# TravisWheelerLab/BATH

Measured on NVIDIA B200. Metric: frameshift Forward GCUPS, higher is better.
Workload: dtype f32

## Files before the change

### bath_b200/csrc/bathgpu.cu

```cuda
#include <cuda_runtime.h>
#include <stdint.h>
#include <stdio.h>
#include <stdarg.h>
#include <string.h>
#include <stdlib.h>
#include <math.h>
#include <thread>
#include <vector>
#include <string>
#include <algorithm>
#include <mutex>
#include <memory>

#include "../../include/bathgpu.h"
#include "fs_parser.cuh"
#include "fs_parser_v3.cuh"
#include "fs_backward.cuh"
#include "fs_domain.cuh"
#include "orf_domain.cuh"
#include "orf_filters.cuh"
#include "orf_finder.cuh"
#include "bias_filter.cuh"
#include "microbench.cuh"
#include "launch.h"
// ... 56 lines not shown
struct FsProfileSet {
  int n = 0;
  std::vector<int> J, scan_steps, mw_scan_steps;
  std::vector<FsSetProfile> table;
  DevBuf arena, dtable, dwins, dwprof, dsc, dst, dcounter;
};

}

struct TargetSlot {
  DevBuf  dna_bytes, dna4, residues, cls;
  int64_t block_n = 0, nres = 0;
  bool    bytes_valid = false;
};
constexpr int kMaxSlots = 1 << 16;

struct bathgpu_ctx {
  int           device = 0;
  cudaDeviceProp prop{};
  cudaStream_t  stream = nullptr, copy_stream = nullptr, stream2 = nullptr;
  cudaStream_t  bulk_stream = nullptr;
  cudaEvent_t   chunk_ev[16] = {};
  cudaEvent_t   ev0 = nullptr, ev1 = nullptr;
  cudaEvent_t   sync_ev = nullptr;
  std::string   err;
  FsProfileImage fs3, fs5;
  FsProfileSet  set3, set5;
  std::vector<std::unique_ptr<TargetSlot>> slot;
  int           cur = 0;
  TargetSlot   &S() { return *slot[cur]; }
  TargetSlot   &slot_at(int i) { while ((int)slot.size() <= i) slot.emplace_back(new TargetSlot()); return *slot[i]; }
  DevBuf        wins, fwdsc, status, counter;
  int           nstaged = 0;
  DevBuf        scratch;
  DevBuf        fxmx, bxmx, lsf, lsb, xoff, dmocc, dbtot, detot, bcksc;
  int64_t       xrows = 0;
  bool          flt_loaded = false;
  bathgpu_filter_params flt{};
  int           flt_W = 0, flt_P = 0;
  DevBuf        f_rbv, f_rwv, f_twv, f_ddsum, f_nrb, orfs, fsc, fst, fwins, fnw;
  DevBuf        b_items, b_tables, b_out;
  DevBuf        o_tiles, o_cnt, o_base, o_blocks, o_first, o_tjb, o_null, o_meta, o_hits, o_counters;
  long long     o_nhits = 0, o_nres = 0;
  cudaEvent_t   o_ev[6] = {};
  float         o_ms[5] = {};
  long long     o_scored = 0, o_norf = 0;
  DevBuf        envs, dpp, doa, dfx, dppx, doax, dlsf, dfw, dbk, doasc, dnull2, dstat, dtoff, dtlen, dsteps, ddcell, dmxout;
  std::vector<long long> dom_xoff;
  std::vector<int>       dom_L;
  float         last_ms = 0.f;
  int           last_launches = 0;
};

static int fail(bathgpu_ctx *ctx, int code, const char *fmt, ...)
{
  char buf[512];
  va_list ap;
  va_start(ap, fmt);
  vsnprintf(buf, sizeof buf, fmt, ap);
  va_end(ap);
  if (ctx) ctx->err = buf;
  return code;
}

#define CUDA_TRY(ctx, call)                                                                      \
  do { cudaError_t e_ = (call);                                                                  \
// ... 766 lines not shown
  const long long p = (long long)blockIdx.x * blockDim.x + threadIdx.x;
  if (p >= n) return;
  const uint8_t comp[18] = { 3, 2, 1, 0, 4, 6, 5, 8, 7, 9, 10, 14, 13, 12, 11, 15, 16, 17 };
  const uint8_t c = src[n - p];
  dst[1 + p] = (c < 18) ? comp[c] : c;
  if (p == 0) { dst[0] = 255; dst[n + 1] = 255; }
}

extern "C" int bathgpu_revcomp_slot(bathgpu_ctx *ctx, int src, int dst)
{
  if (!ctx || src < 0 || src >= kMaxSlots || dst < 0 || dst >= kMaxSlots || src == dst) return fail(ctx, BATHGPU_EINVAL, "bad arguments to bathgpu_revcomp_slot");
  ctx->slot_at(std::max(src, dst));
  TargetSlot &A = *ctx->slot[src], &B = *ctx->slot[dst];
  if (A.block_n == 0) return fail(ctx, BATHGPU_EINVAL, "no block uploaded in slot %d", src);
  CUDA_TRY(ctx, enter(ctx));
  const long long n = A.block_n;
  const long long nwords = (n + 8 + 7) / 8 + 24;
  if (B.dna_bytes.reserve((size_t)n + 2) != BATHGPU_OK || B.dna4.reserve((size_t)nwords * 4) != BATHGPU_OK)
    return fail(ctx, BATHGPU_EMEM, "device allocation failed for a %lld-nt block", n);
  if (!A.bytes_valid) {
    unpack_dna4_kernel<<<(unsigned)(((n + 7) / 8 + 255) / 256), 256, 0, ctx->stream>>>(A.dna4.as<uint32_t>(), n, A.dna_bytes.as<uint8_t>());
    A.bytes_valid = true;
  }
  revcomp_kernel<<<(unsigned)((n + 255) / 256), 256, 0, ctx->stream>>>(A.dna_bytes.as<uint8_t>(), n, B.dna_bytes.as<uint8_t>());
  pack_dna4_kernel<<<(unsigned)((nwords + 255) / 256), 256, 0, ctx->stream>>>(B.dna_bytes.as<uint8_t>(), n, B.dna4.as<uint32_t>(), nwords);
  CUDA_TRY(ctx, cudaGetLastError());
  CUDA_TRY(ctx, wait_stream(ctx));
  B.block_n = n; B.nres = 0; B.bytes_valid = true;
  return BATHGPU_OK;
}


static cudaError_t dispatch_fwd(bool xmx, int J, const FsParserArgs &a, int sms, cudaStream_t s);

static int fs_fwd_block_impl(bathgpu_ctx *ctx, const uint8_t *dsq, const uint8_t *packed, int64_t n, const bathgpu_window *wins, int nwin,
                             const float xfE[2], float *fwdsc, int32_t *status)
{
  if (!ctx || (!dsq && !packed) || n < 1 || !wins || nwin < 1 || !xfE || !fwdsc || !status) return fail(ctx, BATHGPU_EINVAL, "bad arguments to bathgpu_fs_fwd_block");
  if (!ctx->fs3.loaded) return fail(ctx, BATHGPU_EINVAL, "3-codon profile not loaded");
  for (int w = 0; w < nwin; ++w)
    if (wins[w].L < 3 || wins[w].start < 1 || wins[w].start + wins[w].L - 1 > n)
      return fail(ctx, BATHGPU_EINVAL, "window %d (start %lld, L %d) is outside the block (n=%lld) or shorter than 3", w, (long long)wins[w].start, wins[w].L, (long long)n);
  CUDA_TRY(ctx, enter(ctx));
  if (!ctx->copy_stream) {
    CUDA_TRY(ctx, cudaStreamCreateWithFlags(&ctx->copy_stream, cudaStreamNonBlocking));
    CUDA_TRY(ctx, cudaStreamCreateWithFlags(&ctx->stream2, cudaStreamNonBlocking));
    for (auto &e : ctx->chunk_ev) CUDA_TRY(ctx, cudaEventCreateWithFlags(&e, cudaEventDisableTiming));
  }
  TargetSlot &S = ctx->S();
  const long long nwords = (n + 8 + 7) / 8 + 24;
  if (S.dna_bytes.reserve((size_t)n + 2) != BATHGPU_OK || S.dna4.reserve((size_t)nwords * 4) != BATHGPU_OK ||
      ctx->wins.reserve((size_t)nwin * sizeof(WindowDesc)) != BATHGPU_OK || ctx->fwdsc.reserve((size_t)nwin * 4) != BATHGPU_OK ||
      ctx->status.reserve((size_t)nwin * 4) != BATHGPU_OK || ctx->counter.reserve(64) != BATHGPU_OK)
    return fail(ctx, BATHGPU_EMEM, "device allocation failed");
  S.block_n = n; S.nres = 0; S.bytes_valid = (packed == nullptr);
  static_assert(sizeof(WindowDesc) == sizeof(bathgpu_window), "descriptor layouts must agree");
  bool in_order = true;
  for (int w = 1; w < nwin && in_order; ++w) in_order = wins[w - 1].start + wins[w - 1].L <= wins[w].start + wins[w].L;
  std::vector<int> order;
  std::vector<WindowDesc> sorted;
  std::vector<float> sc;
  std::vector<int> st;
  if (!in_order) {
    order.resize((size_t)nwin); sorted.resize((size_t)nwin); sc.resize((size_t)nwin); st.resize((size_t)nwin);
    for (int w = 0; w < nwin; ++w) order[w] = w;
    std::sort(order.begin(), order.end(), [&](int x, int y) { return wins[x].start + wins[x].L < wins[y].start + wins[y].L; });
// ... 3 lines not shown
  long long cuts[8]; int K = 0;
  {
    long long first = n / 85, p = 0;
    const int wave = ctx->prop.multiProcessorCount * 16;
    if (nwin > wave) first = std::min<long long>(std::max<long long>(first, hw[wave].start + hw[wave].L), std::max<long long>(first, n / 8));
    if (n < (4 << 20)) first = n;
    for (long long sz = std::max<long long>(first, 1 << 20); p < n && K < 7; sz *= 4) { p = std::min<long long>(n, (p + sz + 7) & ~7LL); cuts[K++] = p; }
    cuts[K - 1] = n;
  }
  cudaEvent_t *pack_ev = ctx->chunk_ev, *join_ev = ctx->chunk_ev + 8;
  for (int c = 0; c < K; ++c) {
    const long long p0 = c ? cuts[c - 1] : 0, p1 = cuts[c];
    if (packed) {
      CUDA_TRY(ctx, cudaMemcpyAsync(S.dna4.as<uint8_t>() + 4 + p0 / 2, packed + p0 / 2, (size_t)((p1 + 1) / 2 - p0 / 2), cudaMemcpyHostToDevice, ctx->copy_stream));
      {
        const long long b0 = (4 + p0 / 2) & ~127LL, b1 = 4 + (p1 + 1) / 2, lines = (b1 - b0 + 127) / 128;
        l2_prefetch_kernel<<<(unsigned)((lines + 255) / 256), 256, 0, ctx->copy_stream>>>(S.dna4.as<uint8_t>() + b0, b1 - b0);
      }
      if (p1 >= n) dna4_guards_kernel<<<1, 32, 0, ctx->copy_stream>>>(S.dna4.as<uint32_t>(), n);
      else if (c == 0) dna4_guards_kernel<<<1, 1, 0, ctx->copy_stream>>>(S.dna4.as<uint32_t>(), n);
    } else {
      CUDA_TRY(ctx, cudaMemcpyAsync(S.dna_bytes.as<uint8_t>() + 1 + p0, dsq + 1 + p0, (size_t)(p1 - p0), cudaMemcpyHostToDevice, ctx->copy_stream));
      const long long wlo = (c == 0) ? 0 : p0 / 8 + 1, whi = (p1 >= n) ? nwords : p1 / 8 + 1;
      if (whi > wlo)
        pack_dna4_range_kernel<<<(unsigned)((whi - wlo + 255) / 256), 256, 0, ctx->copy_stream>>>(S.dna_bytes.as<uint8_t>(), n, S.dna4.as<uint32_t>(), wlo, whi);
    }
    CUDA_TRY(ctx, cudaGetLastError());
    CUDA_TRY(ctx, cudaEventRecord(pack_ev[c], ctx->copy_stream));
  }
  CUDA_TRY(ctx, cudaMemcpyAsync(ctx->wins.p, hw, (size_t)nwin * sizeof(WindowDesc), cudaMemcpyHostToDevice, ctx->stream));
  CUDA_TRY(ctx, cudaMemsetAsync(ctx->counter.p, 0, 64, ctx->stream));
  CUDA_TRY(ctx, cudaEventRecord(ctx->ev0, ctx->stream));
  const FsProfileImage &im = ctx->fs3;
  int w0 = 0, launches = 0;
  for (int c = 0; c < K; ++c) {
    const long long ready_nt = (c == K - 1) ? n : 8 * (cuts[c] / 8);
    int w1 = w0;
    while (w1 < nwin && hw[w1].start + hw[w1].L - 1 <= ready_nt) ++w1;
    if (c == K - 1) w1 = nwin;
    if (w1 == w0) continue;
    cudaStream_t s = (launches & 1) ? ctx->stream2 : ctx->stream;
    if (launches == 1) CUDA_TRY(ctx, cudaStreamWaitEvent(ctx->stream2, ctx->ev0, 0));
    CUDA_TRY(ctx, cudaStreamWaitEvent(s, pack_ev[c], 0));
    FsParserArgs a{};
    a.emis = im.emis_fwd.as<float>(); a.cellc = im.cellc.as<float>(); a.dna4 = S.dna4.as<uint32_t>();
    a.wins = ctx->wins.as<WindowDesc>() + w0; a.nwin = w1 - w0; a.mpad = im.mpad; a.tEM = xfE[0]; a.tEL = xfE[1];
    a.fwdsc = ctx->fwdsc.as<float>() + w0; a.status = ctx->status.as<int>() + w0; a.xmx = nullptr; a.xoff = nullptr;
    a.counter = ctx->counter.as<int>() + launches; a.scan_steps = im.scan_steps; a.cellmw = im.cellmw.as<float>(); a.mw_scan_steps = im.mw_scan_steps;
    CUDA_TRY(ctx, dispatch_fwd(false, im.J, a, ctx->prop.multiProcessorCount, s));
    ++launches;
    w0 = w1;
  }
  if (launches > 1) {
    CUDA_TRY(ctx, cudaEventRecord(join_ev[0], ctx->stream2));
    CUDA_TRY(ctx, cudaStreamWaitEvent(ctx->stream, join_ev[0], 0));
  }
  CUDA_TRY(ctx, cudaEventRecord(ctx->ev1, ctx->stream));
  CUDA_TRY(ctx, cudaMemcpyAsync(in_order ? fwdsc : sc.data(), ctx->fwdsc.p, (size_t)nwin * 4, cudaMemcpyDeviceToHost, ctx->stream));
  CUDA_TRY(ctx, cudaMemcpyAsync(in_order ? status : st.data(), ctx->status.p, (size_t)nwin * 4, cudaMemcpyDeviceToHost, ctx->stream));
  CUDA_TRY(ctx, wait_stream(ctx));
  CUDA_TRY(ctx, cudaStreamSynchronize(ctx->copy_stream));
  if (!in_order) for (int w = 0; w < nwin; ++w) { fwdsc[order[w]] = sc[w]; status[order[w]] = st[w]; }
  CUDA_TRY(ctx, cudaEventElapsedTime(&ctx->last_ms, ctx->ev0, ctx->ev1));
  ctx->last_launches = launches;
  ctx->nstaged = 0;
  return BATHGPU_OK;
}

extern "C" int bathgpu_fs_fwd_block(bathgpu_ctx *ctx, const uint8_t *dsq, int64_t n, const bathgpu_window *wins, int nwin,
                                    const float xfE[2], float *fwdsc, int32_t *status)
{
  if (!dsq) return fail(ctx, BATHGPU_EINVAL, "bad arguments to bathgpu_fs_fwd_block");
  return fs_fwd_block_impl(ctx, dsq, nullptr, n, wins, nwin, xfE, fwdsc, status);
}

extern "C" int bathgpu_fs_fwd_block_packed4(bathgpu_ctx *ctx, const uint8_t *packed, int64_t n, const bathgpu_window *wins, int nwin,
                                            const float xfE[2], float *fwdsc, int32_t *status)
{
  if (!packed) return fail(ctx, BATHGPU_EINVAL, "bad arguments to bathgpu_fs_fwd_block_packed4");
  return fs_fwd_block_impl(ctx, nullptr, packed, n, wins, nwin, xfE, fwdsc, status);
}

static int fwd_version(int J)
{
  static const int forced = [] { const char *e = getenv("BATHGPU_FWD"); int x = e ? atoi(e) : 0; return (x == 3 || x == 4) ? x : 0; }();
  if (forced) return forced;
  return (J == 10) ? 4 : 3;
}

static cudaError_t dispatch_fwd(bool xmx, int J, const FsParserArgs &a, int sms, cudaStream_t s)
{
  cudaError_t e = cudaErrorInvalidValue;
  const int v = fwd_version(J);
#define X(S) if (launch_fs3_forward_##S(J, xmx, v, a, sms, s, &e)) return e;
  BATHGPU_FOR_EACH_SET(X)
#undef X
  return cudaErrorInvalidValue;
}

static int check_windows(bathgpu_ctx *ctx, const bathgpu_window *wins, int n)
{
  for (int w = 0; w < n; ++w) {
    if (wins[w].L < 3 || wins[w].start < 1 || wins[w].start + wins[w].L - 1 > ctx->S().block_n)
      return fail(ctx, BATHGPU_EINVAL, "window %d (start %lld, L %d) is outside the uploaded block (n=%lld) or shorter than 3",
                  w, (long long)wins[w].start, wins[w].L, (long long)ctx->S().block_n);
  }
  return BATHGPU_OK;
}

extern "C" int bathgpu_stage_windows(bathgpu_ctx *ctx, const bathgpu_window *wins, int n)
{
  if (!ctx || !wins || n < 1) return fail(ctx, BATHGPU_EINVAL, "bad arguments to bathgpu_stage_windows");
  if (ctx->S().block_n == 0)      return fail(ctx, BATHGPU_EINVAL, "no block uploaded");
  int st = check_windows(ctx, wins, n);
  if (st != BATHGPU_OK) return st;
  CUDA_TRY(ctx, enter(ctx));
  static_assert(sizeof(WindowDesc) == sizeof(bathgpu_window), "descriptor layouts must agree");
  if (ctx->wins.reserve((size_t)n * sizeof(WindowDesc)) != BATHGPU_OK || ctx->fwdsc.reserve((size_t)n * 4) != BATHGPU_OK ||
      ctx->status.reserve((size_t)n * 4) != BATHGPU_OK || ctx->counter.reserve(64) != BATHGPU_OK)
    return fail(ctx, BATHGPU_EMEM, "device allocation failed");
  CUDA_TRY(ctx, cudaMemcpyAsync(ctx->wins.p, wins, (size_t)n * sizeof(WindowDesc), cudaMemcpyHostToDevice, ctx->stream));
  CUDA_TRY(ctx, wait_stream(ctx));
  ctx->nstaged = n;
  return BATHGPU_OK;
}

extern "C" int bathgpu_fs_fwd_staged(bathgpu_ctx *ctx, const float xfE[2])
{
  if (!ctx || !xfE)          return fail(ctx, BATHGPU_EINVAL, "bad arguments to bathgpu_fs_fwd_staged");
  if (!ctx->fs3.loaded)      return fail(ctx, BATHGPU_EINVAL, "3-codon profile not loaded");
  if (ctx->nstaged < 1)      return fail(ctx, BATHGPU_EINVAL, "no windows staged");
  CUDA_TRY(ctx, enter(ctx));
  const FsProfileImage &im = ctx->fs3;
  FsParserArgs a{};
  a.emis = im.emis_fwd.as<float>(); a.cellc = im.cellc.as<float>(); a.dna4 = ctx->S().dna4.as<uint32_t>();
  a.wins = ctx->wins.as<WindowDesc>(); a.nwin = ctx->nstaged; a.mpad = im.mpad;
  a.tEM = xfE[0]; a.tEL = xfE[1];
  a.fwdsc = ctx->fwdsc.as<float>(); a.status = ctx->status.as<int>();
  a.xmx = nullptr; a.xoff = nullptr; a.counter = ctx->counter.as<int>(); a.scan_steps = im.scan_steps; a.cellmw = im.cellmw.as<float>(); a.mw_scan_steps = im.mw_scan_steps;

  CUDA_TRY(ctx, cudaMemsetAsync(ctx->counter.p, 0, 4, ctx->stream));
  CUDA_TRY(ctx, cudaEventRecord(ctx->ev0, ctx->stream));
  CUDA_TRY(ctx, dispatch_fwd(false, im.J, a, ctx->prop.multiProcessorCount, ctx->stream));
  CUDA_TRY(ctx, cudaEventRecord(ctx->ev1, ctx->stream));
  CUDA_TRY(ctx, wait_stream(ctx));
  CUDA_TRY(ctx, cudaEventElapsedTime(&ctx->last_ms, ctx->ev0, ctx->ev1));
  ctx->last_launches = 1;
  return BATHGPU_OK;
}

extern "C" int bathgpu_fetch_scores(bathgpu_ctx *ctx, float *fwdsc, int32_t *status, int n)
{
  if (!ctx || n < 1 || n > ctx->nstaged) return fail(ctx, BATHGPU_EINVAL, "bad arguments to bathgpu_fetch_scores");
  CUDA_TRY(ctx, enter(ctx));
  if (fwdsc)  CUDA_TRY(ctx, cudaMemcpyAsync(fwdsc,  ctx->fwdsc.p,  (size_t)n * 4, cudaMemcpyDeviceToHost, ctx->stream));
  if (status) CUDA_TRY(ctx, cudaMemcpyAsync(status, ctx->status.p, (size_t)n * 4, cudaMemcpyDeviceToHost, ctx->stream));
  CUDA_TRY(ctx, wait_stream(ctx));
  return BATHGPU_OK;
}

extern "C" int bathgpu_fs_fwd_windows(bathgpu_ctx *ctx, const bathgpu_window *wins, int n, const float xfE[2],
                                      float *fwdsc, int32_t *status)
{
  int st;
  if (!fwdsc || !status) return fail(ctx, BATHGPU_EINVAL, "bad arguments to bathgpu_fs_fwd_windows");
  if ((st = bathgpu_stage_windows(ctx, wins, n)) != BATHGPU_OK) return st;
  if ((st = bathgpu_fs_fwd_staged(ctx, xfE))     != BATHGPU_OK) return st;
  return bathgpu_fetch_scores(ctx, fwdsc, status, n);
}

static cudaError_t dispatch_bck(int J, const FsBackwardArgs &a, int sms, cudaStream_t s)
{
  cudaError_t e = cudaErrorInvalidValue;
#define X(S) if (launch_fs3_backward_##S(J, a, sms, s, &e)) return e;
  BATHGPU_FOR_EACH_SET(X)
#undef X
  return cudaErrorInvalidValue;
}

static int bck_decode_chunk(bathgpu_ctx *ctx, const bathgpu_window *wins, int n, const float xfE[2], const float xf5_loop[3],
                            const int64_t *out_offset, float *mocc, float *btot, float *etot,
                            float *fwdsc, float *bcksc, int32_t *status,
                            int64_t x_off0 = 0, float *fx_out = nullptr, float *bx_out = nullptr)
{
  const bool decode = (xf5_loop != nullptr);
  const FsProfileImage &im = ctx->fs3;
  std::vector<long long> xoff(n + 1, 0);
  for (int w = 0; w < n; ++w) xoff[w + 1] = xoff[w] + wins[w].L + 1;
  const size_t rows = (size_t)xoff[n];

  if (ctx->wins.reserve((size_t)n * sizeof(WindowDesc)) != BATHGPU_OK || ctx->fwdsc.reserve((size_t)n * 4) != BATHGPU_OK ||
      ctx->bcksc.reserve((size_t)n * 4) != BATHGPU_OK || ctx->status.reserve((size_t)n * 4) != BATHGPU_OK ||
      ctx->counter.reserve(64) != BATHGPU_OK || ctx->xoff.reserve((size_t)(n + 1) * 8) != BATHGPU_OK ||
      ctx->fxmx.reserve(rows * 24) != BATHGPU_OK || ctx->bxmx.reserve(rows * 24) != BATHGPU_OK ||
      ctx->lsf.reserve((rows + 2 * (size_t)n) * 4) != BATHGPU_OK || ctx->lsb.reserve((rows + 2 * (size_t)n) * 4) != BATHGPU_OK ||
      ctx->dmocc.reserve(rows * 4) != BATHGPU_OK || ctx->dbtot.reserve(rows * 4) != BATHGPU_OK || ctx->detot.reserve(rows * 4) != BATHGPU_OK)
    return fail(ctx, BATHGPU_EMEM, "device allocation failed for %d windows (%zu rows)", n, rows);
  CUDA_TRY(ctx, cudaMemcpyAsync(ctx->wins.p, wins, (size_t)n * sizeof(WindowDesc), cudaMemcpyHostToDevice, ctx->stream));
  CUDA_TRY(ctx, cudaMemcpyAsync(ctx->xoff.p, xoff.data(), (size_t)(n + 1) * 8, cudaMemcpyHostToDevice, ctx->stream));
  ctx->nstaged = n;
  ctx->xrows = (int64_t)rows;

  const int sms = ctx->prop.multiProcessorCount;
  CUDA_TRY(ctx, cudaEventRecord(ctx->ev0, ctx->stream));

  FsParserArgs fa{};
  fa.emis = im.emis_fwd.as<float>(); fa.cellc = im.cellc.as<float>(); fa.dna4 = ctx->S().dna4.as<uint32_t>();
  fa.wins = ctx->wins.as<WindowDesc>(); fa.nwin = n; fa.mpad = im.mpad; fa.tEM = xfE[0]; fa.tEL = xfE[1];
  fa.fwdsc = ctx->fwdsc.as<float>(); fa.status = ctx->status.as<int>();
  fa.xmx = ctx->fxmx.as<float>(); fa.xoff = ctx->xoff.as<long long>(); fa.counter = ctx->counter.as<int>(); fa.scan_steps = im.scan_steps; fa.cellmw = im.cellmw.as<float>(); fa.mw_scan_steps = im.mw_scan_steps;
  CUDA_TRY(ctx, cudaMemsetAsync(ctx->counter.p, 0, 4, ctx->stream));
  CUDA_TRY(ctx, dispatch_fwd(true, im.J, fa, sms, ctx->stream));

  FsBackwardArgs ba{};
  ba.emis = im.emis_bck.as<float>(); ba.cellb = im.cellb3.as<float>(); ba.cellbmw = im.cellbmw.as<float>(); ba.dna4 = fa.dna4; ba.wins = fa.wins; ba.nwin = n; ba.mpad = im.mpad;
  ba.tEM = xfE[0]; ba.tEL = xfE[1]; ba.fxmx = ctx->fxmx.as<float>(); ba.bxmx = ctx->bxmx.as<float>(); ba.xoff = fa.xoff;
  ba.bcksc = ctx->bcksc.as<float>(); ba.status = fa.status; ba.counter = fa.counter;
  CUDA_TRY(ctx, cudaMemsetAsync(ctx->counter.p, 0, 4, ctx->stream));
  CUDA_TRY(ctx, dispatch_bck(im.J, ba, sms, ctx->stream));

  std::vector<float> hm, hb, he;
  if (decode) {
    DomainDecodeArgs da{};
    da.fxmx = ba.fxmx; da.bxmx = ba.bxmx; da.xoff = fa.xoff; da.wins = fa.wins; da.nwin = n;
    da.tNL = xf5_loop[0]; da.tJL = xf5_loop[1]; da.tCL = xf5_loop[2];
    da.lsf = ctx->lsf.as<float>(); da.lsb = ctx->lsb.as<float>();
    da.mocc = ctx->dmocc.as<float>(); da.btot = ctx->dbtot.as<float>(); da.etot = ctx->detot.as<float>();
    da.ooff = fa.xoff; da.status = fa.status;
    fs_domain_decoding_kernel<<<(n + 3) / 4, 128, 0, ctx->stream>>>(da);
    CUDA_TRY(ctx, cudaGetLastError());
  }
  CUDA_TRY(ctx, cudaEventRecord(ctx->ev1, ctx->stream));

// ... 343 lines not shown
  for (int p = 0; p < n; ++p) {
    Fold f;
    const int st = fold_profile(ctx, which, M[p], nrows[p], rfv[p], tfv[p], f);
    if (st != BATHGPU_OK) return fail(ctx, st, "profile %d of the set: %s", p, std::string(ctx->err).c_str());
    if (which == 3) forward3_tables(f, 3, nrows[p], rfv[p], tab, cc, mw, ps.scan_steps[p], ps.mw_scan_steps[p]);
    else { emission_table(f, nrows[p], rfv[p], tab); fs5_forward_consts(f, cc); mw.clear(); }
    ps.J[p] = f.J;
    off_emis[p] = append(tab);
    off_cc[p] = append(cc);
    off_mw[p] = mw.empty() ? (size_t)-1 : append(mw);
  }
  CUDA_TRY(ctx, enter(ctx));
  if (ps.arena.reserve(host.size() * sizeof(float)) != BATHGPU_OK || ps.dtable.reserve((size_t)n * sizeof(FsSetProfile)) != BATHGPU_OK)
    return fail(ctx, BATHGPU_EMEM, "device allocation failed for a set of %d profiles (%zu bytes)", n, host.size() * sizeof(float));
  CUDA_TRY(ctx, cudaMemcpyAsync(ps.arena.p, host.data(), host.size() * sizeof(float), cudaMemcpyHostToDevice, ctx->stream));
  CUDA_TRY(ctx, wait_stream(ctx));
  const float *base = ps.arena.as<float>();
  ps.table.assign(n, FsSetProfile{});
  for (int p = 0; p < n; ++p) {
    ps.table[p].emis = base + off_emis[p];
    ps.table[p].cellc = base + off_cc[p];
    ps.table[p].cellmw = (off_mw[p] == (size_t)-1) ? nullptr : base + off_mw[p];
  }
  ps.n = n;
#define X(S) preload_fwd_##S(ps.J[0]); preload_fs5_##S(ps.J[0]);
  BATHGPU_FOR_EACH_SET(X)
#undef X
  return BATHGPU_OK;
}

static cudaError_t dispatch_fwd_set(int J, const FsParserArgs &a, int sms, cudaStream_t s)
{
  cudaError_t e = cudaErrorInvalidValue;
  const int v = fwd_version(J);
#define X(S) if (launch_fs3_forward_set_##S(J, v, a, sms, s, &e)) return e;
  BATHGPU_FOR_EACH_SET(X)
#undef X
  return cudaErrorInvalidValue;
}

static cudaError_t dispatch_fs5_set(int J, const DomainArgs &a, int sms, cudaStream_t s)
{
  cudaError_t e = cudaErrorInvalidValue;
#define X(S) if (launch_fs5_forward_set_##S(J, a, sms, s, &e)) return e;
  BATHGPU_FOR_EACH_SET(X)
#undef X
  return cudaErrorInvalidValue;
}

extern "C" int bathgpu_fs_set_scores(bathgpu_ctx *ctx, int which, const bathgpu_set_window *wins, int n, const float *xfE,
                                     float *fwdsc, int32_t *status)
{
  if (!ctx || !wins || n < 1 || !xfE || !fwdsc || !status) return fail(ctx, BATHGPU_EINVAL, "bad arguments to bathgpu_fs_set_scores");
  if (which != 3 && which != 5) return fail(ctx, BATHGPU_EINVAL, "codon_lengths must be 3 or 5");
  FsProfileSet &ps = (which == 3) ? ctx->set3 : ctx->set5;
  if (ps.n < 1)              return fail(ctx, BATHGPU_EINVAL, "no %d-codon profile set loaded", which);
  if (ctx->S().block_n == 0) return fail(ctx, BATHGPU_EINVAL, "no block uploaded");
  const int minL = (which == 3) ? 3 : 6;
  for (int w = 0; w < n; ++w) {
    if (wins[w].profile < 0 || wins[w].profile >= ps.n)
      return fail(ctx, BATHGPU_EINVAL, "window %d names profile %d of a set of %d", w, wins[w].profile, ps.n);
    if (wins[w].L < minL || wins[w].start < 1 || wins[w].start + wins[w].L - 1 > ctx->S().block_n)
      return fail(ctx, BATHGPU_EINVAL, "window %d (start %lld, L %d) is outside the uploaded block (n=%lld) or shorter than %d",
                  w, (long long)wins[w].start, wins[w].L, (long long)ctx->S().block_n, minL);
  }
  CUDA_TRY(ctx, enter(ctx));
  auto key = [&](int p) -> long long { return which == 3 ? ((long long)ps.J[p] * 8 + ps.scan_steps[p]) * 8 + ps.mw_scan_steps[p] : ps.J[p]; };
// ... 790 lines not shown
```

### bath_b200/csrc/fs_parser.cuh

```cuda
#pragma once
#include <cuda_runtime.h>
#include <stdint.h>

namespace bathgpu {

constexpr int kWarp = 32;

enum FwdCellConst { FC_MM = 0, FC_DM, FC_MD, FC_DD, FC_MI, FC_II, FC_COUNT };
enum FwdLaneConst { FL_B0 = 0, FL_B1, FL_B2, FL_B3, FL_B4, FL_COUNT };

struct WindowDesc {
  long long start;
  int       L;
  float     pmove;
  float     ploop;
};

struct FsSetProfile {
  const float *emis;
  const float *cellc;
  const float *cellmw;
  float        tEM, tEL;
};

struct FsParserArgs {
  const float    *emis;
  const float    *cellc;
  const uint32_t *dna4;
  const WindowDesc *wins;
  int             nwin;
  int             mpad;
  float           tEM, tEL;
  float          *fwdsc;
  int            *status;
  float          *xmx;
  const long long *xoff;
  int            *counter;
  int             scan_steps;
  const float    *cellmw;
  int             mw_scan_steps;
  const FsSetProfile *set;
  const int      *wprof;
};

template <int J> struct VecOf { static constexpr int V = (J % 4 == 0) ? 4 : ((J % 2 == 0) ? 2 : 1); };

__device__ __forceinline__ int codon2_fs3(int w, int x)               { int c = x * 84 + w * 21;                 return min(c, 337); }
__device__ __forceinline__ int codon3_fs3(int v, int w, int x)        { int c = x * 84 + w * 21 + v * 5 + 1;     return min(c, 336); }
__device__ __forceinline__ int codon4_fs3(int u, int v, int w, int x) { int c = x * 84 + w * 21 + v * 5 + u + 2; return min(c, 337); }

template <int J, int VEC>
__device__ __forceinline__ void load_emission_row(const float *__restrict__ row, float (&e)[J])
{
#pragma unroll
  for (int g = 0; g < J / VEC; ++g) {
    if constexpr (VEC == 4) {
      float4 t = __ldg(reinterpret_cast<const float4 *>(row) + g * kWarp);
      e[4 * g + 0] = t.x; e[4 * g + 1] = t.y; e[4 * g + 2] = t.z; e[4 * g + 3] = t.w;
    } else if constexpr (VEC == 2) {
      float2 t = __ldg(reinterpret_cast<const float2 *>(row) + g * kWarp);
      e[2 * g + 0] = t.x; e[2 * g + 1] = t.y;
    } else {
      e[g] = __ldg(row + g * kWarp);
    }
  }
}

__device__ __forceinline__ float warp_allsum(float v)
{
#pragma unroll
  for (int d = 16; d >= 1; d >>= 1) v += __shfl_xor_sync(0xffffffffu, v, d);
  return v;
}

__device__ __forceinline__ void pair_allsum(int lane, float a, float b, float &sa, float &sb)
// ... 167 lines not shown
```

### bath_b200/csrc/kernels_tu.cu

```cuda
#include <algorithm>
#include <cstdlib>
#include "launch.h"
#include "fs_parser.cuh"
#include "fs_parser_v3.cuh"
#include "fs_parser_v4.cuh"
#include "fs_parser_mw.cuh"
#include "fs_backward.cuh"
#include "fs_backward_mw.cuh"
#include "fs_domain.cuh"
#include "orf_domain.cuh"
#include "orf_filters.cuh"

#define FAM_FWD 1
#define FAM_BCK 2
#define FAM_FS5 3
#define FAM_ORF 4
#define FAM_FILT_MSV 5
#define FAM_FILT_VIT_LO 6
#define FAM_FILT_VIT_HI 7

#if   BATHGPU_SET == 0
#define SETNAME a
#define JLIST(X) X(1) X(2) X(3) X(4) X(5)
#elif BATHGPU_SET == 1
#define SETNAME b
#define JLIST(X) X(6) X(7) X(8)
#elif BATHGPU_SET == 2
#define SETNAME c
#define JLIST(X) X(10) X(12)
#elif BATHGPU_SET == 3
#define SETNAME d
#define JLIST(X) X(16)
#elif BATHGPU_SET == 4
#define SETNAME e
#define JLIST(X) X(24)
#elif BATHGPU_SET == 5
#define SETNAME f
#define JLIST(X) X(32)
// ... 5 lines not shown

template <class K> static void touch(K kernel) { cudaFuncAttributes fa; cudaFuncGetAttributes(&fa, kernel); }

template <class K> static int grid_for(K kernel, int threads, size_t smem, int n, int sms)
{
  int nb = 0;
  cudaOccupancyMaxActiveBlocksPerMultiprocessor(&nb, kernel, threads, smem);
  return std::max(1, std::min(n, sms * std::max(nb, 1)));
}

#if BATHGPU_FAMILY == FAM_FWD
template <class K> static int fwd_grid(K kernel, int J, int n, int sms)
{
  static const int env_cap = [] { const char *e = getenv("BATHGPU_FWD_WARPS"); return e ? atoi(e) : 0; }();
  int nb = 0;
  cudaOccupancyMaxActiveBlocksPerMultiprocessor(&nb, kernel, 32, 0);
  const int cap = env_cap > 0 ? env_cap : BATHGPU_V3_RESIDENT(J);
  return std::max(1, std::min(n, sms * std::max(1, std::min(nb, cap))));
}

template <int NW, int JW, bool XMX, bool SET = false> static cudaError_t run_fwd_mw(const FsParserArgs &a, int sms, cudaStream_t s)
{
  if (a.mw_scan_steps <= 3) fs3_forward_parser_kernel_mw<NW, JW, XMX, 3, SET><<<grid_for(fs3_forward_parser_kernel_mw<NW, JW, XMX, 3, SET>, 32 * NW, 0, a.nwin, sms), 32 * NW, 0, s>>>(a);
  else                      fs3_forward_parser_kernel_mw<NW, JW, XMX, 5, SET><<<grid_for(fs3_forward_parser_kernel_mw<NW, JW, XMX, 5, SET>, 32 * NW, 0, a.nwin, sms), 32 * NW, 0, s>>>(a);
  return cudaGetLastError();
}

template <int J, bool XMX, bool SET = false> static cudaError_t run_fwd(int version, const FsParserArgs &a, int sms, cudaStream_t s)
{
  if constexpr (J >= 16) {
    static const int mw_mode = [] { const char *e = getenv("BATHGPU_FWD_MW"); return e ? atoi(e) : 1; }();
    if (version >= 3 && a.cellmw && (mw_mode >= 2 || (mw_mode == 1 && J >= 24))) return run_fwd_mw<J / kMwNodesPerLane, kMwNodesPerLane, XMX, SET>(a, sms, s);
  }
  if (version >= 4) {
    if (a.scan_steps <= 2)      fs3_forward_parser_kernel_v4<J, XMX, 2, SET><<<fwd_grid(fs3_forward_parser_kernel_v4<J, XMX, 2, SET>, J, a.nwin, sms), 32, 0, s>>>(a);
    else if (a.scan_steps == 3) fs3_forward_parser_kernel_v4<J, XMX, 3, SET><<<fwd_grid(fs3_forward_parser_kernel_v4<J, XMX, 3, SET>, J, a.nwin, sms), 32, 0, s>>>(a);
    else                        fs3_forward_parser_kernel_v4<J, XMX, 5, SET><<<fwd_grid(fs3_forward_parser_kernel_v4<J, XMX, 5, SET>, J, a.nwin, sms), 32, 0, s>>>(a);
  }
  else {
    if (a.scan_steps <= 2)      fs3_forward_parser_kernel_v3<J, XMX, 2, SET><<<fwd_grid(fs3_forward_parser_kernel_v3<J, XMX, 2, SET>, J, a.nwin, sms), 32, 0, s>>>(a);
    else if (a.scan_steps == 3) fs3_forward_parser_kernel_v3<J, XMX, 3, SET><<<fwd_grid(fs3_forward_parser_kernel_v3<J, XMX, 3, SET>, J, a.nwin, sms), 32, 0, s>>>(a);
    else                        fs3_forward_parser_kernel_v3<J, XMX, 5, SET><<<fwd_grid(fs3_forward_parser_kernel_v3<J, XMX, 5, SET>, J, a.nwin, sms), 32, 0, s>>>(a);
  }
  return cudaGetLastError();
}
bool CAT(launch_fs3_forward_set_, SETNAME)(int J, int version, const FsParserArgs &a, int sms, cudaStream_t s, cudaError_t *err)
{
  switch (J) {
#define X(J_) case J_: *err = run_fwd<J_, false, true>(version, a, sms, s); return true;
  JLIST(X)
#undef X
  default: return false;
  }
}
bool CAT(launch_fs3_forward_, SETNAME)(int J, bool xmx, int version, const FsParserArgs &a, int sms, cudaStream_t s, cudaError_t *err)
{
  switch (J) {
#define X(J_) case J_: *err = xmx ? run_fwd<J_, true>(version, a, sms, s) : run_fwd<J_, false>(version, a, sms, s); return true;
  JLIST(X)
#undef X
  default: return false;
  }
}
void CAT(preload_fwd_, SETNAME)(int J)
{
  switch (J) {
#define X(J_) case J_: touch(fs3_forward_parser_kernel_v3<J_, false, 2>); touch(fs3_forward_parser_kernel_v3<J_, true, 2>); touch(fs3_forward_parser_kernel_v3<J_, false, 3>); \
                       touch(fs3_forward_parser_kernel_v3<J_, true, 3>); touch(fs3_forward_parser_kernel_v3<J_, false, 5>); touch(fs3_forward_parser_kernel_v3<J_, true, 5>); \
                       if (J_ == 10) { touch(fs3_forward_parser_kernel_v4<J_, false, 2>); touch(fs3_forward_parser_kernel_v4<J_, true, 2>); touch(fs3_forward_parser_kernel_v4<J_, false, 3>); \
                                       touch(fs3_forward_parser_kernel_v4<J_, true, 3>); touch(fs3_forward_parser_kernel_v4<J_, false, 5>); touch(fs3_forward_parser_kernel_v4<J_, true, 5>); } \
                       break;
  JLIST(X)
#undef X
  default: break;
  }
}
#endif

#if BATHGPU_FAMILY == FAM_BCK
template <int J> static cudaError_t run_bck(const FsBackwardArgs &a, int sms, cudaStream_t s)
{
  if constexpr (J >= 16) {
    static const int mw_mode = [] { const char *e = getenv("BATHGPU_BCK_MW"); return e ? atoi(e) : 1; }();
    if (a.cellbmw && mw_mode >= 1) {
      constexpr int NW = J / kMwNodesPerLane;
      fs3_backward_parser_kernel_mw<NW, kMwNodesPerLane><<<grid_for(fs3_backward_parser_kernel_mw<NW, kMwNodesPerLane>, 32 * NW, 0, a.nwin, sms), 32 * NW, 0, s>>>(a);
      return cudaGetLastError();
    }
  }
  fs3_backward_parser_kernel<J><<<grid_for(fs3_backward_parser_kernel<J>, BckTune<J>::kThreads, 0, a.nwin, sms), BckTune<J>::kThreads, 0, s>>>(a);
  return cudaGetLastError();
}
bool CAT(launch_fs3_backward_, SETNAME)(int J, const FsBackwardArgs &a, int sms, cudaStream_t s, cudaError_t *err)
{
  switch (J) {
#define X(J_) case J_: *err = run_bck<J_>(a, sms, s); return true;
  JLIST(X)
#undef X
  default: return false;
  }
}
// ... 230 lines not shown
```

### bath_b200/csrc/launch.h

```cpp
#pragma once
#include <cuda_runtime.h>

namespace bathgpu {

struct FsParserArgs;
struct FsBackwardArgs;
struct DomainArgs;
struct TraceArgs;
struct OrfDomainArgs;
struct OrfFwdArgs;
struct FilterArgs;

#define BATHGPU_FOR_EACH_SET(X) X(a) X(b) X(c) X(d) X(e) X(f)

#define BATHGPU_DECLARE_SET(S)                                                                                                       \
  bool launch_fs3_forward_##S(int J, bool xmx, int version, const FsParserArgs &a, int sms, cudaStream_t s, cudaError_t *err);       \
  bool launch_fs3_backward_##S(int J, const FsBackwardArgs &a, int sms, cudaStream_t s, cudaError_t *err);                           \
  bool launch_fs5_domains_##S(int J, const DomainArgs &a, const TraceArgs &t, int sms, cudaStream_t s, cudaError_t *err);            \
  bool launch_fs5_forward_matrix_##S(int J, const DomainArgs &a, int sms, cudaStream_t s, cudaError_t *err);                         \
  bool launch_orf_domains_##S(int J, bool full, const OrfDomainArgs &a, const TraceArgs &t, int sms, cudaStream_t s, cudaError_t *err); \
  bool launch_orf_forward_matrix_##S(int J, const OrfDomainArgs &a, int sms, cudaStream_t s, cudaError_t *err);                            \
  bool launch_orf_forward_parser_##S(int J, const OrfFwdArgs &a, int sms, cudaStream_t s, cudaError_t *err);                        \
  bool launch_fs3_forward_set_##S(int J, int version, const FsParserArgs &a, int sms, cudaStream_t s, cudaError_t *err);            \
  bool launch_fs5_forward_set_##S(int J, const DomainArgs &a, int sms, cudaStream_t s, cudaError_t *err);                            \
  void preload_fwd_##S(int J); void preload_bck_##S(int J); void preload_fs5_##S(int J); void preload_orf_##S(int J);
BATHGPU_FOR_EACH_SET(BATHGPU_DECLARE_SET)
#undef BATHGPU_DECLARE_SET

constexpr int kMwNodesPerLane = 8;

bool launch_msv_filter(int W, int P, int mode, const FilterArgs &a, int sms, cudaStream_t s, cudaError_t *err);
bool launch_vit_filter_lo(int P, const FilterArgs &a, int sms, cudaStream_t s, cudaError_t *err);
bool launch_vit_filter_hi(int P, const FilterArgs &a, int sms, cudaStream_t s, cudaError_t *err);
void preload_msv_filter(int W, int P); void preload_vit_filter_lo(int P); void preload_vit_filter_hi(int P);

}
```

Measured before the change: 1339.

## Add paired-window v5 forward kernel with length-sorted window ordering

Adds a new forward parser kernel in which each warp processes two windows at once, packing their states into float2 so the arithmetic runs on paired FMA operations. Windows are counting-sorted by quad length on the host so the paired windows have similar lengths and little padding is wasted. The kernel is selected by default only when J==6 (or when forced through an environment variable). In exchange it raises register pressure and adds a small host sort and an extra order-array transfer per launch.

```diff
diff --git a/bath_b200/csrc/bathgpu.cu b/bath_b200/csrc/bathgpu.cu
--- a/bath_b200/csrc/bathgpu.cu
+++ b/bath_b200/csrc/bathgpu.cu
@@ -112,6 +112,8 @@
   TargetSlot   &slot_at(int i) { while ((int)slot.size() <= i) slot.emplace_back(new TargetSlot()); return *slot[i]; }
   DevBuf        wins, fwdsc, status, counter;
   int           nstaged = 0;
+  DevBuf        worder;
+  bool          staged_order = false;
   DevBuf        scratch;
   DevBuf        fxmx, bxmx, lsf, lsb, xoff, dmocc, dbtot, detot, bcksc;
   int64_t       xrows = 0;
@@ -944,6 +946,8 @@
 
 
 static cudaError_t dispatch_fwd(bool xmx, int J, const FsParserArgs &a, int sms, cudaStream_t s);
+static int fwd_version(int J, bool xmx);
+static bool order_by_quads(const WindowDesc *wins, int n, int *order);
 
 static int fs_fwd_block_impl(bathgpu_ctx *ctx, const uint8_t *dsq, const uint8_t *packed, int64_t n, const bathgpu_window *wins, int nwin,
                              const float xfE[2], float *fwdsc, int32_t *status)
@@ -1013,6 +1017,9 @@
   CUDA_TRY(ctx, cudaMemsetAsync(ctx->counter.p, 0, 64, ctx->stream));
   CUDA_TRY(ctx, cudaEventRecord(ctx->ev0, ctx->stream));
   const FsProfileImage &im = ctx->fs3;
+  const bool pairs = fwd_version(im.J, false) == 5;
+  std::vector<int> worder(pairs ? (size_t)nwin : 0);
+  if (pairs && ctx->worder.reserve((size_t)nwin * 4) != BATHGPU_OK) return fail(ctx, BATHGPU_EMEM, "device allocation failed");
   int w0 = 0, launches = 0;
   for (int c = 0; c < K; ++c) {
     const long long ready_nt = (c == K - 1) ? n : 8 * (cuts[c] / 8);
@@ -1023,11 +1030,14 @@
     cudaStream_t s = (launches & 1) ? ctx->stream2 : ctx->stream;
     if (launches == 1) CUDA_TRY(ctx, cudaStreamWaitEvent(ctx->stream2, ctx->ev0, 0));
     CUDA_TRY(ctx, cudaStreamWaitEvent(s, pack_ev[c], 0));
+    const bool ordered = pairs && order_by_quads(hw + w0, w1 - w0, worder.data() + w0);
+    if (ordered) CUDA_TRY(ctx, cudaMemcpyAsync(ctx->worder.as<int>() + w0, worder.data() + w0, (size_t)(w1 - w0) * 4, cudaMemcpyHostToDevice, s));
     FsParserArgs a{};
     a.emis = im.emis_fwd.as<float>(); a.cellc = im.cellc.as<float>(); a.dna4 = S.dna4.as<uint32_t>();
     a.wins = ctx->wins.as<WindowDesc>() + w0; a.nwin = w1 - w0; a.mpad = im.mpad; a.tEM = xfE[0]; a.tEL = xfE[1];
     a.fwdsc = ctx->fwdsc.as<float>() + w0; a.status = ctx->status.as<int>() + w0; a.xmx = nullptr; a.xoff = nullptr;
     a.counter = ctx->counter.as<int>() + launches; a.scan_steps = im.scan_steps; a.cellmw = im.cellmw.as<float>(); a.mw_scan_steps = im.mw_scan_steps;
+    a.order = ordered ? ctx->worder.as<int>() + w0 : nullptr;
     CUDA_TRY(ctx, dispatch_fwd(false, im.J, a, ctx->prop.multiProcessorCount, s));
     ++launches;
     w0 = w1;
@@ -1045,6 +1055,7 @@
   CUDA_TRY(ctx, cudaEventElapsedTime(&ctx->last_ms, ctx->ev0, ctx->ev1));
   ctx->last_launches = launches;
   ctx->nstaged = 0;
+  ctx->staged_order = false;
   return BATHGPU_OK;
 }
 
@@ -1062,17 +1073,31 @@
   return fs_fwd_block_impl(ctx, nullptr, packed, n, wins, nwin, xfE, fwdsc, status);
 }
 
-static int fwd_version(int J)
-{
-  static const int forced = [] { const char *e = getenv("BATHGPU_FWD"); int x = e ? atoi(e) : 0; return (x == 3 || x == 4) ? x : 0; }();
+static int fwd_version(int J, bool xmx)
+{
+  static const int forced = [] { const char *e = getenv("BATHGPU_FWD"); int x = e ? atoi(e) : 0; return (x >= 3 && x <= 5) ? x : 0; }();
+  const bool pairs = !xmx && fwd_pairs_kernel(J);
+  if (forced == 5 || (!forced && J == 6)) return pairs ? 5 : 3;
   if (forced) return forced;
   return (J == 10) ? 4 : 3;
 }
 
+static bool order_by_quads(const WindowDesc *wins, int n, int *order)
+{
+  int lo = INT32_MAX, hi = 0;
+  for (int w = 0; w < n; ++w) { const int q = (wins[w].L + 4) >> 2; lo = std::min(lo, q); hi = std::max(hi, q); }
+  if (n < 3 || lo == hi) return false;
+  std::vector<int> pos((size_t)(hi - lo) + 2, 0);
+  for (int w = 0; w < n; ++w) ++pos[((wins[w].L + 4) >> 2) - lo + 1];
+  for (size_t q = 1; q < pos.size(); ++q) pos[q] += pos[q - 1];
+  for (int w = 0; w < n; ++w) order[pos[((wins[w].L + 4) >> 2) - lo]++] = w;
+  return true;
+}
+
 static cudaError_t dispatch_fwd(bool xmx, int J, const FsParserArgs &a, int sms, cudaStream_t s)
 {
   cudaError_t e = cudaErrorInvalidValue;
-  const int v = fwd_version(J);
+  const int v = fwd_version(J, xmx);
 #define X(S) if (launch_fs3_forward_##S(J, xmx, v, a, sms, s, &e)) return e;
   BATHGPU_FOR_EACH_SET(X)
 #undef X
@@ -1097,12 +1122,17 @@
   if (st != BATHGPU_OK) return st;
   CUDA_TRY(ctx, enter(ctx));
   static_assert(sizeof(WindowDesc) == sizeof(bathgpu_window), "descriptor layouts must agree");
+  std::vector<int> order((size_t)n);
+  const bool ordered = order_by_quads(reinterpret_cast<const WindowDesc *>(wins), n, order.data());
   if (ctx->wins.reserve((size_t)n * sizeof(WindowDesc)) != BATHGPU_OK || ctx->fwdsc.reserve((size_t)n * 4) != BATHGPU_OK ||
-      ctx->status.reserve((size_t)n * 4) != BATHGPU_OK || ctx->counter.reserve(64) != BATHGPU_OK)
+      ctx->status.reserve((size_t)n * 4) != BATHGPU_OK || ctx->counter.reserve(64) != BATHGPU_OK ||
+      (ordered && ctx->worder.reserve((size_t)n * 4) != BATHGPU_OK))
     return fail(ctx, BATHGPU_EMEM, "device allocation failed");
   CUDA_TRY(ctx, cudaMemcpyAsync(ctx->wins.p, wins, (size_t)n * sizeof(WindowDesc), cudaMemcpyHostToDevice, ctx->stream));
+  if (ordered) CUDA_TRY(ctx, cudaMemcpyAsync(ctx->worder.p, order.data(), (size_t)n * 4, cudaMemcpyHostToDevice, ctx->stream));
   CUDA_TRY(ctx, wait_stream(ctx));
   ctx->nstaged = n;
+  ctx->staged_order = ordered;
   return BATHGPU_OK;
 }
 
@@ -1119,6 +1149,7 @@
   a.tEM = xfE[0]; a.tEL = xfE[1];
   a.fwdsc = ctx->fwdsc.as<float>(); a.status = ctx->status.as<int>();
   a.xmx = nullptr; a.xoff = nullptr; a.counter = ctx->counter.as<int>(); a.scan_steps = im.scan_steps; a.cellmw = im.cellmw.as<float>(); a.mw_scan_steps = im.mw_scan_steps;
+  a.order = ctx->staged_order ? ctx->worder.as<int>() : nullptr;
 
   CUDA_TRY(ctx, cudaMemsetAsync(ctx->counter.p, 0, 4, ctx->stream));
   CUDA_TRY(ctx, cudaEventRecord(ctx->ev0, ctx->stream));
@@ -1180,6 +1211,7 @@
   CUDA_TRY(ctx, cudaMemcpyAsync(ctx->wins.p, wins, (size_t)n * sizeof(WindowDesc), cudaMemcpyHostToDevice, ctx->stream));
   CUDA_TRY(ctx, cudaMemcpyAsync(ctx->xoff.p, xoff.data(), (size_t)(n + 1) * 8, cudaMemcpyHostToDevice, ctx->stream));
   ctx->nstaged = n;
+  ctx->staged_order = false;
   ctx->xrows = (int64_t)rows;
 
   const int sms = ctx->prop.multiProcessorCount;
@@ -1589,7 +1621,7 @@
 static cudaError_t dispatch_fwd_set(int J, const FsParserArgs &a, int sms, cudaStream_t s)
 {
   cudaError_t e = cudaErrorInvalidValue;
-  const int v = fwd_version(J);
+  const int v = fwd_version(J, true);
 #define X(S) if (launch_fs3_forward_set_##S(J, v, a, sms, s, &e)) return e;
   BATHGPU_FOR_EACH_SET(X)
 #undef X
diff --git a/bath_b200/csrc/fs_parser.cuh b/bath_b200/csrc/fs_parser.cuh
--- a/bath_b200/csrc/fs_parser.cuh
+++ b/bath_b200/csrc/fs_parser.cuh
@@ -41,6 +41,7 @@
   int             mw_scan_steps;
   const FsSetProfile *set;
   const int      *wprof;
+  const int      *order;
 };
 
 template <int J> struct VecOf { static constexpr int V = (J % 4 == 0) ? 4 : ((J % 2 == 0) ? 2 : 1); };
diff --git a/bath_b200/csrc/fs_parser_v5.cuh b/bath_b200/csrc/fs_parser_v5.cuh
--- /dev/null
+++ b/bath_b200/csrc/fs_parser_v5.cuh
@@ -0,0 +1,218 @@
+#pragma once
+#include "fs_parser_v4.cuh"
+
+namespace bathgpu {
+
+template <int J>
+struct FwdState5 {
+  float2 W[4][J], I[4][J];
+  float2 xN[4], xJ[4], xC[4];
+};
+
+__device__ __forceinline__ float2 shfl_up2(float2 v, int d)
+{
+  return make_float2(__shfl_up_sync(0xffffffffu, v.x, d), __shfl_up_sync(0xffffffffu, v.y, d));
+}
+
+__device__ __forceinline__ float2 warp_allsum2(float2 v)
+{
+#pragma unroll
+  for (int d = 16; d >= 1; d >>= 1) v = fadd2(v, make_float2(__shfl_xor_sync(0xffffffffu, v.x, d), __shfl_xor_sync(0xffffffffu, v.y, d)));
+  return v;
+}
+
+template <int J, int VEC, int PH, int NS, bool HEAD>
+__device__ __forceinline__ float2 fwd5_row(int iA, int iB, int lane, FwdState5<J> &S, const FwdConsts<J> &K,
+                                           const char *__restrict__ emis_lane, unsigned rowbytes, uint32_t cwA, uint32_t cwB,
+                                           float2 ploop, float2 pmove, float tEL, float tEM)
+{
+  constexpr int P0 = PH, P1 = (PH + 3) & 3, P2 = (PH + 2) & 3, P3 = (PH + 1) & 3;
+  float a2[J], a3[J], a4[J], b2[J], b3[J], b4[J];
+  float2 m[J];
+  load_emission_row<J, VEC>(reinterpret_cast<const float *>(emis_lane + (size_t)(cwA & 511u) * rowbytes), a2);
+  load_emission_row<J, VEC>(reinterpret_cast<const float *>(emis_lane + (size_t)((cwA >> 9) & 511u) * rowbytes), a3);
+  load_emission_row<J, VEC>(reinterpret_cast<const float *>(emis_lane + (size_t)(cwA >> 18) * rowbytes), a4);
+  load_emission_row<J, VEC>(reinterpret_cast<const float *>(emis_lane + (size_t)(cwB & 511u) * rowbytes), b2);
+  load_emission_row<J, VEC>(reinterpret_cast<const float *>(emis_lane + (size_t)((cwB >> 9) & 511u) * rowbytes), b3);
+  load_emission_row<J, VEC>(reinterpret_cast<const float *>(emis_lane + (size_t)(cwB >> 18) * rowbytes), b4);
+
+  float2 es0 = make_float2(0.f, 0.f), es1 = make_float2(0.f, 0.f);
+#pragma unroll
+  for (int j = 0; j < J; ++j) {
+    float2 t = fmul2(S.W[P2][j], make_float2(a4[j], b4[j]));
+    t = ffma2(S.W[P1][j], make_float2(a3[j], b3[j]), t);
+    t = ffma2(S.W[P0][j], make_float2(a2[j], b2[j]), t);
+    m[j] = t;
+    const float2 q = bcast2(K.qm[j]);
+    if (j == 0) es0 = fmul2(t, q); else if (j == 1) es1 = fmul2(t, q); else if (j & 1) es1 = ffma2(t, q, es1); else es0 = ffma2(t, q, es0);
+  }
+  const float2 xE = warp_allsum2(J > 1 ? fadd2(es0, es1) : es0);
+
+  float2 A = m[0];
+#pragma unroll
+  for (int j = 1; j < J; ++j) A = ffma2(A, bcast2(K.dd[j]), m[j]);
+#pragma unroll
+  for (int s = 0; s < NS; ++s) A = ffma2(bcast2(K.bs[s]), shfl_up2(A, 1 << s), A);
+  float2 d = shfl_up2(A, 1);
+
+  float2 xN = fmul2(S.xN[P3], ploop);
+  if constexpr (HEAD) {
+    xN.x = (iA < 3) ? ((iA >= 0) ? 1.0f : 0.0f) : xN.x;
+    xN.y = (iB < 3) ? ((iB >= 0) ? 1.0f : 0.0f) : xN.y;
+  }
+  const float2 xJ = ffma2(S.xJ[P3], ploop, fmul2(xE, bcast2(tEL)));
+  const float2 xC = ffma2(S.xC[P3], ploop, fmul2(xE, bcast2(tEM)));
+  const float2 xB = ffma2(xJ, pmove, fmul2(xN, pmove));
+
+  float2 o[J];
+#pragma unroll
+  for (int j = 0; j < J; ++j) {
+    const float2 t = ffma2(S.I[P0][j], bcast2(K.hi[j]), m[j]);
+    o[j] = ffma2(d, bcast2(K.dm[j]), t);
+    if (j + 1 < J) d = ffma2(d, bcast2(K.dd[j]), m[j]);
+    S.I[P1][j] = ffma2(S.I[P0][j], bcast2(K.ii[j]), m[j]);
+  }
+  float2 oprev = shfl_up2(o[J - 1], 1);
+  if (lane == 0) oprev = make_float2(0.f, 0.f);
+  S.W[P2][0] = fadd2(xB, oprev);
+#pragma unroll
+  for (int j = 1; j < J; ++j) S.W[P2][j] = fadd2(xB, o[j - 1]);
+  S.xN[P0] = xN; S.xJ[P0] = xJ; S.xC[P0] = xC;
+  return xE;
+}
+
+template <int J>
+__device__ __forceinline__ void scale_state5(FwdState5<J> &S, float2 sf)
+{
+#pragma unroll
+  for (int r = 0; r < 4; ++r) {
+#pragma unroll
+    for (int j = 0; j < J; ++j) { S.W[r][j] = fmul2(S.W[r][j], sf); S.I[r][j] = fmul2(S.I[r][j], sf); }
+    S.xN[r] = fmul2(S.xN[r], sf); S.xJ[r] = fmul2(S.xJ[r], sf); S.xC[r] = fmul2(S.xC[r], sf);
+  }
+}
+
+__device__ __forceinline__ float2 rescale_factors5(float2 xE, float2 &totscale)
+{
+  float2 sf = make_float2(1.0f, 1.0f);
+  if (xE.x > 1.0e4f) { sf.x = 1.0f / xE.x; totscale.x += logf(xE.x); }
+  if (xE.y > 1.0e4f) { sf.y = 1.0f / xE.y; totscale.y += logf(xE.y); }
+  return sf;
+}
+
+template <int J, int VEC, int PH, int NS, bool HEAD>
+__device__ __forceinline__ void fwd5_row_pair(int iA, int iB, int lane, FwdState5<J> &S, const FwdConsts<J> &K,
+                                              const char *__restrict__ emis_lane, unsigned rowbytes,
+                                              uint32_t cwA0, uint32_t cwB0, uint32_t cwA1, uint32_t cwB1,
+                                              float2 ploop, float2 pmove, float tEL, float tEM, float2 &totscale)
+{
+  const float2 E0 = fwd5_row<J, VEC, PH, NS, HEAD>(iA, iB, lane, S, K, emis_lane, rowbytes, cwA0, cwB0, ploop, pmove, tEL, tEM);
+  float2 E1 = fwd5_row<J, VEC, PH + 1, NS, HEAD>(iA + 1, iB + 1, lane, S, K, emis_lane, rowbytes, cwA1, cwB1, ploop, pmove, tEL, tEM);
+  if (__builtin_expect(fmaxf(fmaxf(E0.x, E0.y), fmaxf(E1.x, E1.y)) > 1.0e4f, 0)) {
+    if (E0.x > 1.0e4f || E0.y > 1.0e4f) {
+      const float2 sf = rescale_factors5(E0, totscale);
+      scale_state5<J>(S, sf);
+      E1 = fmul2(E1, sf);
+    }
+    if (E1.x > 1.0e4f || E1.y > 1.0e4f) scale_state5<J>(S, rescale_factors5(E1, totscale));
+  }
+}
+
+#ifndef BATHGPU_V5_WARPS
+#define BATHGPU_V5_WARPS(J) 8
+#endif
+
+__device__ __forceinline__ void load_dna_pair(const uint32_t *__restrict__ dna4, long long nib, uint32_t &lo, uint32_t &hi)
+{
+  lo = (nib >= 0) ? __ldg(dna4 + (nib >> 3)) : 0u;
+  hi = (nib >= -8) ? __ldg(dna4 + (nib >> 3) + 1) : 0u;
+}
+
+template <int J, int NS = 5>
+__global__ void __launch_bounds__(32, BATHGPU_V5_WARPS(J)) fs3_forward_parser_kernel_v5(FsParserArgs a)
+{
+  constexpr int VEC = VecOf<J>::V;
+  const int lane = threadIdx.x & 31;
+
+  FwdConsts<J> K;
+  load_fwd_consts<J>(a.cellc, lane, K);
+  const char    *emis_lane = reinterpret_cast<const char *>(a.emis + lane * VEC);
+  const float    tEM = a.tEM, tEL = a.tEL;
+  const unsigned rowbytes = (unsigned)a.mpad * 4u;
+
+  for (;;) {
+    int k = 0;
+    if (lane == 0) k = atomicAdd(a.counter, 2);
+    k = __shfl_sync(0xffffffffu, k, 0);
+    if (k >= a.nwin) break;
+    int wA = k, wB = (k + 1 < a.nwin) ? k + 1 : k;
+    if (a.order) { wA = a.order[wA]; wB = a.order[wB]; }
+
+    const WindowDesc da = a.wins[wA], db = a.wins[wB];
+    const int    LA = da.L, LB = db.L;
+    const float2 pmove = make_float2(da.pmove, db.pmove), ploop = make_float2(da.ploop, db.ploop);
+
+    FwdState5<J> S;
+#pragma unroll
+    for (int r = 0; r < 4; ++r) {
+#pragma unroll
+      for (int j = 0; j < J; ++j) { S.W[r][j] = make_float2(0.f, 0.f); S.I[r][j] = make_float2(0.f, 0.f); }
+      S.xN[r] = make_float2(0.f, 0.f); S.xJ[r] = make_float2(0.f, 0.f); S.xC[r] = make_float2(0.f, 0.f);
+    }
+    float2 totscale = make_float2(0.f, 0.f);
+
+    const int nq   = max((LA + 4) >> 2, (LB + 4) >> 2);
+    const int padA = 4 * nq - (LA + 1), padB = 4 * nq - (LB + 1);
+    const int padmax = max(padA, padB);
+    long long nibA = (da.start - 1) + (long long)(lane - padA - 3) - 1 + 8;
+    long long nibB = (db.start - 1) + (long long)(lane - padB - 3) - 1 + 8;
+    uint32_t loA, hiA, loB, hiB;
+    load_dna_pair(a.dna4, nibA, loA, hiA);
+    load_dna_pair(a.dna4, nibB, loB, hiB);
+    int iA = -padA, iB = -padB;
+
+#define BATHGPU_V5_CHUNK(HEAD_)                                                                                                   \
+    {                                                                                                                             \
+      const uint32_t cwlA = codon_word(loA, hiA, (int)(nibA & 7) * 4, iA + lane, LA);                                             \
+      const uint32_t cwlB = codon_word(loB, hiB, (int)(nibB & 7) * 4, iB + lane, LB);                                             \
+      nibA += 32; nibB += 32;                                                                                                     \
+      if (q0 + 8 < nq) { load_dna_pair(a.dna4, nibA, loA, hiA); load_dna_pair(a.dna4, nibB, loB, hiB); }                          \
+      const int qn = min(8, nq - q0);                                                                                             \
+      for (int qq = 0; qq < qn; ++qq) {                                                                                           \
+        const uint32_t a0 = __shfl_sync(0xffffffffu, cwlA, qq * 4 + 0), b0 = __shfl_sync(0xffffffffu, cwlB, qq * 4 + 0);           \
+        const uint32_t a1 = __shfl_sync(0xffffffffu, cwlA, qq * 4 + 1), b1 = __shfl_sync(0xffffffffu, cwlB, qq * 4 + 1);           \
+        const uint32_t a2 = __shfl_sync(0xffffffffu, cwlA, qq * 4 + 2), b2 = __shfl_sync(0xffffffffu, cwlB, qq * 4 + 2);           \
+        const uint32_t a3 = __shfl_sync(0xffffffffu, cwlA, qq * 4 + 3), b3 = __shfl_sync(0xffffffffu, cwlB, qq * 4 + 3);           \
+        fwd5_row_pair<J, VEC, 0, NS, HEAD_>(iA, iB, lane, S, K, emis_lane, rowbytes, a0, b0, a1, b1, ploop, pmove, tEL, tEM, totscale); \
+        iA += 2; iB += 2;                                                                                                         \
+        fwd5_row_pair<J, VEC, 2, NS, HEAD_>(iA, iB, lane, S, K, emis_lane, rowbytes, a2, b2, a3, b3, ploop, pmove, tEL, tEM, totscale); \
+        iA += 2; iB += 2;                                                                                                         \
+      }                                                                                                                           \
+    }
+    int q0 = 0;
+    for (; q0 < nq && 4 * q0 < padmax + 3; q0 += 8) BATHGPU_V5_CHUNK(true)
+    for (; q0 < nq; q0 += 8) BATHGPU_V5_CHUNK(false)
+#undef BATHGPU_V5_CHUNK
+
+    {
+      float tot = S.xC[3].x + S.xC[2].x * ploop.x + S.xC[1].x * ploop.x;
+      int   st  = 0;
+      float sc;
+      if (isnan(tot) || isinf(tot))   { st = 16; sc = tot; }
+      else if (LA > 2 && tot == 0.0f) { st = 16; sc = -INFINITY; }
+      else sc = totscale.x + logf(tot * pmove.x);
+      if (lane == 0) { a.fwdsc[wA] = sc; a.status[wA] = st; }
+    }
+    if (wB != wA) {
+      float tot = S.xC[3].y + S.xC[2].y * ploop.y + S.xC[1].y * ploop.y;
+      int   st  = 0;
+      float sc;
+      if (isnan(tot) || isinf(tot))   { st = 16; sc = tot; }
+      else if (LB > 2 && tot == 0.0f) { st = 16; sc = -INFINITY; }
+      else sc = totscale.y + logf(tot * pmove.y);
+      if (lane == 0) { a.fwdsc[wB] = sc; a.status[wB] = st; }
+    }
+  }
+}
+
+}
diff --git a/bath_b200/csrc/kernels_tu.cu b/bath_b200/csrc/kernels_tu.cu
--- a/bath_b200/csrc/kernels_tu.cu
+++ b/bath_b200/csrc/kernels_tu.cu
@@ -4,6 +4,7 @@
 #include "fs_parser.cuh"
 #include "fs_parser_v3.cuh"
 #include "fs_parser_v4.cuh"
+#include "fs_parser_v5.cuh"
 #include "fs_parser_mw.cuh"
 #include "fs_backward.cuh"
 #include "fs_backward_mw.cuh"
@@ -75,7 +76,16 @@
     static const int mw_mode = [] { const char *e = getenv("BATHGPU_FWD_MW"); return e ? atoi(e) : 1; }();
     if (version >= 3 && a.cellmw && (mw_mode >= 2 || (mw_mode == 1 && J >= 24))) return run_fwd_mw<J / kMwNodesPerLane, kMwNodesPerLane, XMX, SET>(a, sms, s);
   }
-  if (version >= 4) {
+  if constexpr (fwd_pairs_kernel(J) && !XMX && !SET) {
+    if (version == 5) {
+      const int npair = (a.nwin + 1) / 2;
+      if (a.scan_steps <= 2)      fs3_forward_parser_kernel_v5<J, 2><<<fwd_grid(fs3_forward_parser_kernel_v5<J, 2>, J, npair, sms), 32, 0, s>>>(a);
+      else if (a.scan_steps == 3) fs3_forward_parser_kernel_v5<J, 3><<<fwd_grid(fs3_forward_parser_kernel_v5<J, 3>, J, npair, sms), 32, 0, s>>>(a);
+      else                        fs3_forward_parser_kernel_v5<J, 5><<<fwd_grid(fs3_forward_parser_kernel_v5<J, 5>, J, npair, sms), 32, 0, s>>>(a);
+      return cudaGetLastError();
+    }
+  }
+  if (version == 4) {
     if (a.scan_steps <= 2)      fs3_forward_parser_kernel_v4<J, XMX, 2, SET><<<fwd_grid(fs3_forward_parser_kernel_v4<J, XMX, 2, SET>, J, a.nwin, sms), 32, 0, s>>>(a);
     else if (a.scan_steps == 3) fs3_forward_parser_kernel_v4<J, XMX, 3, SET><<<fwd_grid(fs3_forward_parser_kernel_v4<J, XMX, 3, SET>, J, a.nwin, sms), 32, 0, s>>>(a);
     else                        fs3_forward_parser_kernel_v4<J, XMX, 5, SET><<<fwd_grid(fs3_forward_parser_kernel_v4<J, XMX, 5, SET>, J, a.nwin, sms), 32, 0, s>>>(a);
@@ -110,6 +120,8 @@
   switch (J) {
 #define X(J_) case J_: touch(fs3_forward_parser_kernel_v3<J_, false, 2>); touch(fs3_forward_parser_kernel_v3<J_, true, 2>); touch(fs3_forward_parser_kernel_v3<J_, false, 3>); \
                        touch(fs3_forward_parser_kernel_v3<J_, true, 3>); touch(fs3_forward_parser_kernel_v3<J_, false, 5>); touch(fs3_forward_parser_kernel_v3<J_, true, 5>); \
+                       if constexpr (fwd_pairs_kernel(J_)) { touch(fs3_forward_parser_kernel_v5<J_, 2>); touch(fs3_forward_parser_kernel_v5<J_, 3>); \
+                                                             touch(fs3_forward_parser_kernel_v5<J_, 5>); } \
                        if (J_ == 10) { touch(fs3_forward_parser_kernel_v4<J_, false, 2>); touch(fs3_forward_parser_kernel_v4<J_, true, 2>); touch(fs3_forward_parser_kernel_v4<J_, false, 3>); \
                                        touch(fs3_forward_parser_kernel_v4<J_, true, 3>); touch(fs3_forward_parser_kernel_v4<J_, false, 5>); touch(fs3_forward_parser_kernel_v4<J_, true, 5>); } \
                        break;
diff --git a/bath_b200/csrc/launch.h b/bath_b200/csrc/launch.h
--- a/bath_b200/csrc/launch.h
+++ b/bath_b200/csrc/launch.h
@@ -29,6 +29,8 @@
 
 constexpr int kMwNodesPerLane = 8;
 
+constexpr bool fwd_pairs_kernel(int J) { return J == 5 || J == 6; }
+
 bool launch_msv_filter(int W, int P, int mode, const FilterArgs &a, int sms, cudaStream_t s, cudaError_t *err);
 bool launch_vit_filter_lo(int P, const FilterArgs &a, int sms, cudaStream_t s, cudaError_t *err);
 bool launch_vit_filter_hi(int P, const FilterArgs &a, int sms, cudaStream_t s, cudaError_t *err);
```

After: 1058 (median of 6 runs). -21.0%, worse.
